# scverse/muon

Measured on AMD Instinct MI355X. Metric: cells/sec for TF-IDF+LSI(k=50), higher is better.
Workload: dtype f32

## Files before the change

### include/muon_amd.h

```cpp
#ifndef MUON_AMD_H
#define MUON_AMD_H

#include <stddef.h>
#include <stdint.h>

#ifdef __cplusplus
extern "C" {
#endif

typedef enum {
  MU_OK = 0,
  MU_ERR_ARG = -1,
  MU_ERR_HIP = -2,
  MU_ERR_NO_DEVICE = -3,
  MU_ERR_UNSUPPORTED = -4
} mu_status;

#define MU_DTYPE_F32 0
#define MU_DTYPE_F64 1

#define MU_TFIDF_LOG_TF 1
#define MU_TFIDF_LOG_IDF 2
#define MU_TFIDF_LOG_TFIDF 4

// ... 56 lines not shown
                                const float* d_values, const double* d_rowsum, const float* d_idf, double scale,
                                int flags, float* d_out, unsigned long long* d_zero_count, void* d_work,
                                size_t work_bytes, int have_slab_ptr, const int64_t* d_slab_ptr,
                                const int64_t* d_row_dst, void* d_ent, void* stream);
int mu_csr_slab_ptr(int64_t n_rows, int64_t n_cols, const int64_t* d_indptr, const int32_t* d_indices, int64_t* d_sp,
                    void* stream);
int mu_csr_slab_ptr_width(int64_t n_rows, int64_t n_cols, int64_t width, const int64_t* d_indptr,
                          const int32_t* d_indices, int64_t* d_sp, void* stream);
int mu_csr_row_col_sums_sp(int dtype, int64_t n_rows, int64_t n_cols, const int64_t* d_indptr,
                           const int32_t* d_indices, const void* d_values, double* d_rowsum, double* d_colsum,
                           void* d_work, size_t work_bytes, const int64_t* d_slab_ptr, void* stream);
int mu_tfidf_scale_sweep_sp(int dtype, int64_t n_rows, int64_t n_cols, const int64_t* d_indptr,
                            const int32_t* d_indices, const void* d_values, const double* d_rowsum, const void* d_idf,
                            double scale, int flags, void* d_out, unsigned long long* d_zero_count,
                            const int64_t* d_slab_ptr, void* stream);
int mu_tpack4_supported(int64_t n_rows, int64_t n_cols, int64_t nnz);
int mu_tpack4_geometry(int64_t n_rows, int64_t n_cols, int64_t nnz, int64_t* rows_per_block, int* n_blocks,
                       int* tile_cols);
size_t mu_tpack4_worksize(int64_t n_rows, int64_t n_cols, int64_t nnz);
int mu_tpack4_count(int64_t n_rows, int64_t n_cols, int64_t nnz, const int64_t* d_indptr, const int32_t* d_indices,
                    int64_t* d_col_nnz, void* d_work, size_t work_bytes, const int64_t* d_slab_ptr, void* stream);
int mu_tpack4_fill_stream(int64_t n_rows, int64_t n_cols, int64_t nnz, const int64_t* d_indptr,
                          const int32_t* d_indices, const float* d_values, const int64_t* d_x_row_dst,
                          const void* d_x_ent, const int64_t* d_sptr, const int32_t* d_inv, void* d_ent, void* d_work,
                          size_t work_bytes, void* stream);
int mu_tpack4_fill_csr(int64_t n_rows, int64_t n_cols, int64_t nnz, const int64_t* d_indptr, const int32_t* d_indices,
                       const float* d_values, const int64_t* d_x_row_dst, const void* d_x_ent,
                       const int64_t* d_t_indptr, int32_t* d_t_indices, float* d_t_values, void* d_work,
                       size_t work_bytes, void* stream);
int mu_tpack4_status(const void* d_work, int64_t n_rows, int64_t n_cols, int64_t nnz, int* h_err);
size_t mu_tpack4_err_offset(int64_t n_rows, int64_t n_cols, int64_t nnz);
size_t mu_tpack4_cnt_offset(int64_t n_rows, int64_t n_cols, int64_t nnz);
int mu_tpack4_phase_cycles(unsigned long long* h_out6, int reset);
int mu_csr_stream_len(int64_t n_pos, const int32_t* d_perm, const int64_t* d_indptr, int64_t* d_len,
                      void* stream);
int mu_csr_stream_fill(int64_t n_pos, const int32_t* d_perm, const int64_t* d_indptr,
                       const int32_t* d_indices, const float* d_values, const int64_t* d_sptr,
                       void* d_ent, void* stream);
int mu_spmm_stream_f32(int64_t n_pos, int64_t n_cols, const int64_t* d_sptr, const void* d_ent,
                       const int32_t* d_perm, int k_layout, const float* d_Q, int B, float* d_Y,
                       void* stream);
int mu_csr_slice_stream(int n_ranges, const int64_t* h_row0, const int64_t* h_rows, const int64_t* h_lo,
                        const int64_t* h_hi, int64_t n_cols, const int64_t* d_indptr, const int32_t* d_indices,
                        const float* d_values, const int64_t* d_slab_ptr, int64_t* d_sptr, void* d_ent, uint32_t* d_rel,
                        void* stream);
int mu_spmm_stream_ranges_f32(int64_t n_pos, const int64_t* d_sptr, const void* d_ent, const int32_t* d_perm,
                              int k_layout, const float* d_Q, int64_t q_rows, float* d_Y, int64_t y_stride,
                              const uint32_t* d_tbl, int64_t tbl_stride, int n_ranges, const int32_t* h_ranges5,
                              int per_wg, void* stream);
int mu_spmm_stream_f64(int64_t n_pos, int64_t n_cols, const int64_t* d_sptr, const void* d_ent,
                       const int32_t* d_perm, int k_layout, const double* d_Q, int B, double* d_Y,
                       int accumulate, void* stream);


int mu_spmm_ell16_waves(int64_t n_rows);
int mu_spmm_ell16_f32(int waves, int64_t n_pos, int64_t n_cols, const int32_t* d_hdr, const int64_t* d_wave_base,
                      const void* d_ent, const int32_t* d_perm, const float* d_Q, float* d_Y, void* stream);
int mu_spmm_ell16_f64(int waves, int64_t n_pos, int64_t n_cols, const int32_t* d_hdr, const int64_t* d_wave_base,
                      const void* d_ent, const int32_t* d_perm, const double* d_Q, double* d_Y, int accumulate,
                      void* stream);
int mu_spmm_ell16_parts(int64_t n_rows, int64_t n_cols, int wide, int* waves, int* parts);
int mu_spmm_ell16_parts_f32(int waves, int parts, int64_t n_pos, int64_t n_cols, const int32_t* d_hdr,
                            const int64_t* d_wave_base, const void* d_ent, const int32_t* d_perm, const float* d_Q,
                            float* d_Y, int64_t y_stride, void* stream);
int mu_spmm_ell16_parts_f64(int waves, int parts, int64_t n_pos, int64_t n_cols, const int32_t* d_hdr,
                            const int64_t* d_wave_base, const void* d_ent, const int32_t* d_perm, const double* d_Q,
// ... 135 lines not shown
```

### muon_amd/_backend.py

```python
from __future__ import annotations

from dataclasses import dataclass
from typing import Optional, Tuple

import contextlib
import os

import numpy as np
import torch

from . import _ffi
from ._ffi import F32, F64, check


@dataclass
class DeviceCSR:

    indptr: torch.Tensor
    indices: torch.Tensor
    values: torch.Tensor
    shape: Tuple[int, int]

    @property
    def nnz(self) -> int:
# ... 594 lines not shown
        self._tpack4_err = work[off:off + 4].view(torch.int32).clone()

    def take_tpack4_err(self):
        return self.__dict__.pop("_tpack4_err", None)

    @staticmethod
    def raise_tpack4(err: int) -> None:
        if int(err) != 0:
            raise _ffi.MuonAmdError(f"mu_tpack4_fill: the transposition tripped an internal invariant (error word {int(err)}: "
                                    "1 = bitmap and count pass disagree, 2 = a tile could not be narrowed); X^T would be wrong")

    def tpack4_status(self) -> int:
        import ctypes as C

        got = self.__dict__.get("_tpack4_work")
        if got is None:
            return 0
        work, (n, d, nnz) = got
        err = C.c_int(0)
        check(self.lib.mu_tpack4_status(_p(work), n, d, nnz, C.byref(err)))
        return int(err.value)

    def transpose_stream(self, X: DeviceCSR, sort_rows: bool = True, before_fill=None,
                         K: Optional[int] = None, src=None) -> DeviceStream:
        n, d = X.shape
        assert X.values.dtype == torch.float32
        col_nnz = self.empty((max(d, 1),), torch.int64)
        plan = self._plan_of(X, "tplan") if (sort_rows and K is None and self._use_tpack4(X)) else None
        if plan is not None:
            ent = self.empty((max(X.nnz, 1),), torch.int64)
            if before_fill is not None:
                before_fill()
            xs_ent, xs_dst = (src[0].ent, src[1]) if src is not None else (None, None)
            with self._dev_ctx():
                check(self.lib.mu_tpack4_fill_stream(n, d, X.nnz, _p(X.indptr), _p(X.indices), _p(X.values),
                                                     _p(xs_dst), _p(xs_ent), _p(plan["sptr"]), _p(plan["inv"]), _p(ent),
                                                     _p(plan["work"]), plan["wb"], self._stream()))
            self._note_tpack4(plan["work"], n, d, X.nnz)
            return DeviceStream(plan["sptr"], ent, (d, n), X.nnz, plan["perm"], plan["K"], self._t4_prefix(plan["work"], n, d, X.nnz))
        if self._use_tpack4(X):
            wb = int(self.lib.mu_tpack4_worksize(n, d, X.nnz))
            work = self.empty((wb,), torch.uint8)
            with self._dev_ctx():
                st = self._stream()
                check(self.lib.mu_tpack4_count(n, d, X.nnz, _p(X.indptr), _p(X.indices), _p(col_nnz), _p(work), wb,
                                               _p(self._slab_ptr_of(X)), st))
                want_k = K
                perm, inv, K, n_pos = None, None, max(1, int(want_k or self.lib.mu_spmm_stream_k(d))), d
                lens = col_nnz[:d]
                if sort_rows and d > 0:
                    perm, inv, K = self.launch_layout(lens, want_k)
                    n_pos = int(perm.numel())
                    plens = torch.zeros((n_pos,), dtype=torch.int64, device=self.device)
                    plens[inv.long()] = lens
                else:
                    plens = lens.contiguous()
                sptr = self._stream_sptr(plens, K)
                ent = self.empty((max(X.nnz, 1),), torch.int64)
                if before_fill is not None:
                    before_fill()
                xs_ent, xs_dst = (src[0].ent, src[1]) if src is not None else (None, None)
                check(self.lib.mu_tpack4_fill_stream(n, d, X.nnz, _p(X.indptr), _p(X.indices), _p(X.values),
                                                     _p(xs_dst), _p(xs_ent), _p(sptr), _p(inv), _p(ent), _p(work), wb, st))
            self._note_tpack4(work, n, d, X.nnz)
            return DeviceStream(sptr, ent, (d, n), X.nnz, perm, K, self._t4_prefix(work, n, d, X.nnz))
        if before_fill is not None:
            before_fill()
        return self.stream(self.transpose(X), sort_rows=sort_rows, K=K)

    def _t4_geometry(self, n, d, nnz):
        import ctypes as C

        rpb, G, Ct = C.c_int64(0), C.c_int(0), C.c_int(0)
        check(self.lib.mu_tpack4_geometry(n, d, nnz, C.byref(rpb), C.byref(G), C.byref(Ct)))
        return int(rpb.value), int(G.value)

    def _t4_prefix(self, work, n, d, nnz):
        rpb, G = self._t4_geometry(n, d, nnz)
        off = int(self.lib.mu_tpack4_cnt_offset(n, d, nnz))
        cnt = work[off:off + 4 * (G + 1) * d].view(torch.int32)
        return dict(cnt=cnt, rpb=rpb, blocks=G, stride=d)

    def slice_plan(self, X: DeviceCSR, n_s: int, max_ranges: int = 16):
        n, d = X.shape
        if n_s <= 0 or X.values.dtype != torch.float32 or not self._use_tpack4(X) or self._slab_ptr_of(X) is None:
            return None
        key = (X.indptr.data_ptr(), X.indices.data_ptr(), n, d, X.nnz, int(n_s), int(max_ranges))
        shared = self._plan_of(X, "tplan")
        got = shared.get("wplan") if shared is not None else getattr(X, "wplan", None)
        if got is not None and got[1] == key:
            return got[0]
        rpb, G = self._t4_geometry(n, d, X.nnz)
        if G < 1:
            return None
        blocks = max(1, min(G, int(round(n_s / rpb))))
        R = max(1, min(int(max_ranges), blocks))
        per = max(1, min(int(round(blocks / R)), G // R))
        g0s = [(r * G) // R for r in range(R)]
        rows = [(g0 * rpb, min((g0 + per) * rpb, n)) for g0 in g0s]
        edges = X.indptr[torch.tensor([v for ab in rows for v in ab], device=X.indptr.device)].tolist()
        plan = dict(rpb=rpb, ranges=[dict(g0=g0, g1=g0 + per, row0=a, row1=b, lo=int(edges[2 * i]), hi=int(edges[2 * i + 1]))
# ... 647 lines not shown
```

### muon_amd/_ffi.py

```python
from __future__ import annotations

import ctypes as C
import os
import threading

_HERE = os.path.dirname(os.path.abspath(__file__))
LIB_PATH = os.path.join(_HERE, "csrc", "libmuon_amd.so")

F32, F64 = 0, 1
TFIDF_LOG_TF, TFIDF_LOG_IDF, TFIDF_LOG_TFIDF = 1, 2, 4


class MuonAmdError(RuntimeError):
    pass


_lib = None
_lock = threading.Lock()

_i64, _i32, _dbl, _vp, _sz, _u64 = C.c_int64, C.c_int, C.c_double, C.c_void_p, C.c_size_t, C.c_uint64

SIGNATURES = {
    "mu_version": (C.c_int, []),
    "mu_last_error": (C.c_char_p, []),
# ... 13 lines not shown
    "mu_tfidf_scale": (C.c_int, [_i32, _i64, _vp, _vp, _vp, _vp, _vp, _dbl, _i32, _vp, _vp, _vp]),
    "mu_tfidf_scale_sweep": (C.c_int, [_i32, _i64, _i64, _vp, _vp, _vp, _vp, _vp, _dbl, _i32, _vp, _vp, _vp,
                                       _sz, _i32, _vp]),
    "mu_csr_count_nonzero": (C.c_int, [_i32, _i64, _vp, _vp, _vp, _vp]),
    "mu_csr_compact_nonzero": (C.c_int, [_i32, _i64, _vp, _vp, _vp, _vp, _vp, _vp, _vp]),
    "mu_exclusive_scan_i64": (C.c_int, [_i64, _vp, _vp, _vp]),
    "mu_binarize_values": (C.c_int, [_i32, _i64, _vp, _vp]),
    "mu_csr_transpose_worksize": (_sz, [_i64, _i64, _i64]),
    "mu_csr_transpose": (C.c_int, [_i32, _i64, _i64, _i64, _vp, _vp, _vp, _vp, _vp, _vp, _vp, _sz, _vp]),
    "mu_spmm_f32": (C.c_int, [_i64, _i64, _vp, _vp, _vp, _vp, _i32, _vp, _i32, _vp]),
    "mu_spmm_stream_k": (C.c_int, [_i64]),
    "mu_tfidf_scale_sweep_stream": (C.c_int, [_i64, _i64, _vp, _vp, _vp, _vp, _vp, _dbl, _i32, _vp, _vp, _vp, _sz, _i32,
                                              _vp, _vp, _vp, _vp]),
    "mu_csr_slab_ptr": (C.c_int, [_i64, _i64, _vp, _vp, _vp, _vp]),
    "mu_csr_slab_ptr_width": (C.c_int, [_i64, _i64, _i64, _vp, _vp, _vp, _vp]),
    "mu_csr_row_col_sums_sp": (C.c_int, [_i32, _i64, _i64, _vp, _vp, _vp, _vp, _vp, _vp, _sz, _vp, _vp]),
    "mu_tfidf_scale_sweep_sp": (C.c_int, [_i32, _i64, _i64, _vp, _vp, _vp, _vp, _vp, _dbl, _i32, _vp, _vp, _vp, _vp]),
    "mu_tpack4_supported": (C.c_int, [_i64, _i64, _i64]),
    "mu_tpack4_geometry": (C.c_int, [_i64, _i64, _i64, C.POINTER(_i64), C.POINTER(C.c_int), C.POINTER(C.c_int)]),
    "mu_tpack4_worksize": (_sz, [_i64, _i64, _i64]),
    "mu_tpack4_count": (C.c_int, [_i64, _i64, _i64, _vp, _vp, _vp, _vp, _sz, _vp, _vp]),
    "mu_tpack4_fill_stream": (C.c_int, [_i64, _i64, _i64, _vp, _vp, _vp, _vp, _vp, _vp, _vp, _vp, _vp, _sz, _vp]),
    "mu_tpack4_fill_csr": (C.c_int, [_i64, _i64, _i64, _vp, _vp, _vp, _vp, _vp, _vp, _vp, _vp, _vp, _sz, _vp]),
    "mu_tpack4_status": (C.c_int, [_vp, _i64, _i64, _i64, C.POINTER(C.c_int)]),
    "mu_tpack4_err_offset": (_sz, [_i64, _i64, _i64]),
    "mu_tpack4_phase_cycles": (C.c_int, [_vp, _i32]),
    "mu_csr_stream_len": (C.c_int, [_i64, _vp, _vp, _vp, _vp]),
    "mu_csr_stream_fill": (C.c_int, [_i64, _vp, _vp, _vp, _vp, _vp, _vp, _vp]),
    "mu_spmm_stream_f32": (C.c_int, [_i64, _i64, _vp, _vp, _vp, _i32, _vp, _i32, _vp, _vp]),
    "mu_spmm_stream_f64": (C.c_int, [_i64, _i64, _vp, _vp, _vp, _i32, _vp, _i32, _vp, _i32, _vp]),
    "mu_csr_slice_stream": (C.c_int, [_i32, _vp, _vp, _vp, _vp, _i64, _vp, _vp, _vp, _vp, _vp, _vp, _vp, _vp]),
    "mu_spmm_stream_ranges_f32": (C.c_int, [_i64, _vp, _vp, _vp, _i32, _vp, _i64, _vp, _i64, _vp, _i64, _i32, _vp, _i32, _vp]),
    "mu_tpack4_cnt_offset": (_sz, [_i64, _i64, _i64]),
    "mu_spmm_ell16_waves": (C.c_int, [_i64]),
    "mu_dense_col_moments_chunks": (C.c_int, [_i64, _i64]),
    "mu_dense_col_moments": (C.c_int, [_i32, _i64, _i64, _i64, _vp, _i32, _vp, _vp]),
    "mu_ell16_fill": (C.c_int, [_i64, _i64, _i64, _i32, _vp, _vp, _vp, _vp, _vp, _vp, _vp, _vp]),
    "mu_spmm_ell16_f32": (C.c_int, [_i32, _i64, _i64, _vp, _vp, _vp, _vp, _vp, _vp, _vp]),
    "mu_spmm_ell16_f64": (C.c_int, [_i32, _i64, _i64, _vp, _vp, _vp, _vp, _vp, _vp, _i32, _vp]),
    "mu_spmm_ell16_parts": (C.c_int, [_i64, _i64, _i32, C.POINTER(C.c_int), C.POINTER(C.c_int)]),
    "mu_spmm_ell16_parts_f32": (C.c_int, [_i32, _i32, _i64, _i64, _vp, _vp, _vp, _vp, _vp, _vp, _i64, _vp]),
    "mu_spmm_ell16_parts_f64": (C.c_int, [_i32, _i32, _i64, _i64, _vp, _vp, _vp, _vp, _vp, _vp, _i64, _vp]),
    "mu_tune_set": (C.c_int, [C.c_char_p, _i32]),
    "mu_tune_get": (C.c_int, [C.c_char_p]),
    "mu_spmm_f64": (C.c_int, [_i64, _i64, _vp, _vp, _vp, _vp, _i32, _vp, _i32, _vp]),
    "mu_gram_worksize": (_sz, [_i64, _i32]),
    "mu_gram_f32": (C.c_int, [_i64, _i32, _vp, _vp, _vp, _vp, _sz, _vp]),
    "mu_gram_cross_f32": (C.c_int, [_i64, _i32, _vp, _vp, _vp, _vp, _sz, _vp]),
    "mu_dense_apply_f32": (C.c_int, [_i64, _i32, _vp, _vp, _vp, _vp, _vp]),
    "mu_dense_project_out_f32": (C.c_int, [_i64, _i32, _vp, _vp, _vp, _vp]),
    "mu_chol_rinv_f64": (C.c_int, [_i32, _i32, _vp, _vp, _vp, _vp]),
    "mu_randn_f32": (C.c_int, [_i64, _u64, _vp, _vp]),
    "mu_skinny_tn_worksize": (_sz, [_i32, _i64, _i64]),
    "mu_skinny_nn": (C.c_int, [_i32, _i64, _i64, _i64, _vp, _vp, _vp, _vp]),
    "mu_skinny_tn": (C.c_int, [_i32, _i64, _i64, _i64, _vp, _vp, _vp, _vp, _sz, _vp]),
    "mu_skinny_nn_f64_f32": (C.c_int, [_i64, _i64, _i64, _vp, _vp, _vp, _vp]),
    "mu_skinny_tn_f64_f32": (C.c_int, [_i64, _i64, _i64, _vp, _vp, _vp, _vp, _sz, _vp]),
    "mu_mofa_update_w": (C.c_int, [_i32, _i64, _i32, _i32] + [_vp] * 7 + [_i32] + [_vp] * 6),
    "mu_mofa_update_z": (C.c_int, [_i32, _i64, _i32, _i32, _i32] + [_vp] * 11),
    "mu_mofa_rowstats_work_doubles": (_sz, [_i32]),
    "mu_mofa_rowstats": (C.c_int, [_i32, _i64, _i64, _i32, _vp, _vp, _vp, _vp, _i32, _vp, _i32, _i32, _vp, _i64,
                                   _vp, _vp, _vp, _vp, _vp]),
    "mu_umap_strengths_f64": (C.c_int, [_i64, _i32, _vp, _vp, _dbl, _dbl, _vp, _vp]),
    "mu_wnn_bandwidth_f64": (C.c_int, [_i64, _i32, _vp, _vp, _vp, _vp, _vp, _i32, _dbl, _vp, _vp, _vp]),
    "mu_knn_filter_f64": (C.c_int, [_i64, _i64, _i64, _i32] + [_vp] * 6 + [_i32] + [_vp] * 4),
    "mu_knn_merge_f64": (C.c_int, [_i64, _i32, _i32] + [_vp] * 9),
# ... 72 lines not shown
```

### muon_amd/csrc/build.py

```python
#!/usr/bin/env python
import hashlib
import os
import subprocess
import sys

HERE = os.path.dirname(os.path.abspath(__file__))
ROOT = os.path.dirname(os.path.dirname(HERE))
SOURCES = ["runtime.hip", "tfidf.hip", "transpose.hip", "spmm.hip", "spmm_win.hip", "spmm_narrow.hip", "spmm_ell.hip", "tpack4.hip", "dense.hip", "skinny.hip", "synth.hip", "mofa.hip", "mofa_elbo.hip", "mofa_stats.hip", "mofa_poisson.hip", "mofa_bernoulli.hip", "knn.hip", "wnn.hip"]
HEADERS = ["common.hpp", "sweep.hpp", os.path.join(ROOT, "include", "muon_amd.h")]
_VGPR_FORM = ["-mllvm", "-amdgpu-mfma-vgpr-form"]
EXTRA = {"skinny.hip": _VGPR_FORM, "dense.hip": _VGPR_FORM, "knn.hip": _VGPR_FORM, "mofa_poisson.hip": _VGPR_FORM, "mofa_bernoulli.hip": _VGPR_FORM}
LIB = os.path.join(HERE, "libmuon_amd.so")
ARCH = "gfx950"
FLAGS = ["-O3", "-std=c++17", "-fPIC", f"--offload-arch={ARCH}", "-I" + os.path.join(ROOT, "include"),
         "-I" + HERE, "-Wall", "-Wno-unused-function"]


def _hipcc():
    for cand in (os.environ.get("HIPCC"), "/opt/rocm/bin/hipcc", "hipcc"):
        if cand and (os.path.isabs(cand) and os.path.exists(cand) or not os.path.isabs(cand)):
            return cand
    raise RuntimeError("hipcc not found")


def _digest(paths):
    h = hashlib.sha256()
    for p in paths:
        with open(p, "rb") as f:
            h.update(f.read())
    h.update(" ".join(f for f in FLAGS if not f.startswith("-I")).encode())
    h.update(repr(sorted(EXTRA.items())).encode())
    h.update(_compiler_id().encode())
    return h.hexdigest()


def _compiler_id():
    try:
        out = subprocess.run([_hipcc(), "--version"], capture_output=True, text=True, timeout=30).stdout
        return " | ".join(l.strip() for l in out.splitlines() if "version" in l.lower())[:300]
    except Exception:
        return ""
# ... 36 lines not shown
```

### muon_amd/csrc/runtime.hip

```cpp
#include <atomic>
#include <cstdarg>
#include <cstdio>
#include <cstring>
#include <thread>
#include <vector>
#include "common.hpp"

static thread_local char g_err[512] = "";

void mu_set_error(const char* fmt, ...) {
  va_list ap;
  va_start(ap, fmt);
  vsnprintf(g_err, sizeof(g_err), fmt, ap);
  va_end(ap);
}

int mu_num_cus() {
  static int cached[64] = {0};
  int dev = 0;
  if (hipGetDevice(&dev) != hipSuccess || dev < 0 || dev >= 64) return 256;
  if (cached[dev] == 0) {
    int n = 0;
    if (hipDeviceGetAttribute(&n, hipDeviceAttributeMultiprocessorCount, dev) != hipSuccess ||
        n <= 0)
      n = 256;
    cached[dev] = n;
  }
  return cached[dev];
}

static const char* const kTuneKeys[] = {"spmm_k", "spmm_mode", "gram_wg", "pack_wg", "tpack_dbg", "spmm_narrow_off", "ell_mode", "tfidf_wide", "tfidf_pipe", "nn_interleave", "tfidf_abl", "tfidf_sum_m", "tn_pipe", "nn_fast_off", "stream_pipe", "tpack4_m", "tpack4_c", "scale_stream_off", "tpack4_plain", "tpack4_abl", "tpack4_late", "tpack4_circ", "tpack4_off", "pois_valu", "pois_lane"};
constexpr int kTuneN = sizeof(kTuneKeys) / sizeof(kTuneKeys[0]);
static int g_tune[kTuneN] = {};

extern "C" {

int mu_version(void) { return 601; }

int mu_tune_set(const char* key, int value) {
  MU_REQUIRE(key, "null key");
  for (int i = 0; i < kTuneN; ++i)
    if (strcmp(key, kTuneKeys[i]) == 0) {
      MU_REQUIRE(value >= 0, "negative value");
      MU_REQUIRE(i != 0 || value <= 16, "spmm_k must be 0..16");
      g_tune[i] = value;
      return MU_OK;
    }
  mu_set_error("mu_tune_set: unknown key %s", key);
  return MU_ERR_ARG;
}

int mu_tune_get(const char* key) {
  if (key)
    for (int i = 0; i < kTuneN; ++i)
      if (strcmp(key, kTuneKeys[i]) == 0) return g_tune[i];
  return -1;
}

const char* mu_last_error(void) { return g_err; }

int mu_device_count(int* count) {
  MU_REQUIRE(count, "null count");
  int n = 0;
  hipError_t e = hipGetDeviceCount(&n);
// ... 120 lines not shown
```

Before: 3.450 million.

## Add precomputed tile permutation plan for transpose-stream fill from row stream

Adds a new tperm kernel pair. A one-time plan pass records column tiles, overflow continuation lanes and per-entry staging slots. A move kernel then transposes the already-packed row stream of X into the column stream using those cached slots, with inline-asm pipelined loads and a double-buffered LDS staging area. The goal is to skip the per-call counting, sorting and bitmap work of the tpack4 fill when the plan is reused across calls. The cost is extra memory for the plan (a 16-bit slot per nnz), heavy register-pinned inline assembly, and a fallback path when alignment or plan preconditions fail.

```diff
diff --git a/include/muon_amd.h b/include/muon_amd.h
--- a/include/muon_amd.h
+++ b/include/muon_amd.h
@@ -112,6 +112,13 @@
 size_t mu_tpack4_err_offset(int64_t n_rows, int64_t n_cols, int64_t nnz);
 size_t mu_tpack4_cnt_offset(int64_t n_rows, int64_t n_cols, int64_t nnz);
 int mu_tpack4_phase_cycles(unsigned long long* h_out6, int reset);
+int mu_tperm_stage_pairs(void);
+int mu_tperm_plan(int64_t n_rows, int64_t n_cols, int64_t nnz, const int64_t* d_indptr, const int32_t* d_indices,
+                  const int64_t* d_x_row_dst, int tile_cols, const int64_t* d_tile_off, int32_t* d_ntile,
+                  int32_t* d_tiles, uint32_t* d_cont, uint16_t* d_slots, void* stream);
+int mu_tperm_fill(int64_t n_rows, int64_t n_cols, int64_t nnz, const int64_t* d_indptr, const int64_t* d_x_row_dst,
+                  const void* d_x_ent, const int64_t* d_cdst, const void* d_cnt, const int64_t* d_tile_off,
+                  const int32_t* d_tiles, const uint32_t* d_cont, const uint16_t* d_slots, void* d_ent, void* stream);
 int mu_csr_stream_len(int64_t n_pos, const int32_t* d_perm, const int64_t* d_indptr, int64_t* d_len,
                       void* stream);
 int mu_csr_stream_fill(int64_t n_pos, const int32_t* d_perm, const int64_t* d_indptr,
diff --git a/muon_amd/_backend.py b/muon_amd/_backend.py
--- a/muon_amd/_backend.py
+++ b/muon_amd/_backend.py
@@ -650,10 +650,17 @@
             if before_fill is not None:
                 before_fill()
             xs_ent, xs_dst = (src[0].ent, src[1]) if src is not None else (None, None)
+            tp = self._tperm_of(X, plan, xs_ent, xs_dst) if src is not None else None
             with self._dev_ctx():
-                check(self.lib.mu_tpack4_fill_stream(n, d, X.nnz, _p(X.indptr), _p(X.indices), _p(X.values),
-                                                     _p(xs_dst), _p(xs_ent), _p(plan["sptr"]), _p(plan["inv"]), _p(ent),
-                                                     _p(plan["work"]), plan["wb"], self._stream()))
+                if tp is not None:
+                    cnt = plan["work"][int(self.lib.mu_tpack4_cnt_offset(n, d, X.nnz)):]
+                    check(self.lib.mu_tperm_fill(n, d, X.nnz, _p(X.indptr), _p(xs_dst), _p(xs_ent), _p(tp["cdst"]), _p(cnt),
+                                                 _p(tp["toff"]), _p(tp["tiles"]), _p(tp["cont"]), _p(tp["slots"]), _p(ent),
+                                                 self._stream()))
+                else:
+                    check(self.lib.mu_tpack4_fill_stream(n, d, X.nnz, _p(X.indptr), _p(X.indices), _p(X.values),
+                                                         _p(xs_dst), _p(xs_ent), _p(plan["sptr"]), _p(plan["inv"]), _p(ent),
+                                                         _p(plan["work"]), plan["wb"], self._stream()))
             self._note_tpack4(plan["work"], n, d, X.nnz)
             return DeviceStream(plan["sptr"], ent, (d, n), X.nnz, plan["perm"], plan["K"], self._t4_prefix(plan["work"], n, d, X.nnz))
         if self._use_tpack4(X):
@@ -685,6 +692,46 @@
         if before_fill is not None:
             before_fill()
         return self.stream(self.transpose(X), sort_rows=sort_rows, K=K)
+
+    def _tperm_of(self, X: DeviceCSR, plan, xs_ent, xs_dst):
+        import ctypes as C
+
+        lib = self.lib
+        if plan.get("tperm") is False:
+            return None
+        xplan = self._plan_of(X, "xplan")
+        if (lib.mu_tune_get(b"tperm_off") == 1 or lib.mu_tune_get(b"tpack_dbg") > 0 or xplan is None
+                or xs_dst is not xplan["row_dst"] or xs_ent.data_ptr() % 256 != 0):
+            return None
+        n, d = X.shape
+        got = plan.get("tperm")
+        keys = (lib.mu_tune_get(b"tpack4_c"), lib.mu_tune_get(b"tpack4_m"))
+        if got is not None and got["keys"] == keys:
+            return got
+        rpb, G, Ct = C.c_int64(0), C.c_int(0), C.c_int(0)
+        check(lib.mu_tpack4_geometry(n, d, X.nnz, C.byref(rpb), C.byref(G), C.byref(Ct)))
+        G, Ct = int(G.value), min(int(Ct.value), 512)
+        try:
+            with self._dev_ctx():
+                st = self._stream()
+                ntile = self.empty((G,), torch.int32)
+                check(lib.mu_tperm_plan(n, d, X.nnz, _p(X.indptr), _p(X.indices), None, Ct, None, _p(ntile), None, None,
+                                        None, st))
+                toff = torch.zeros((G + 1,), dtype=torch.int64, device=self.device)
+                toff[1:] = torch.cumsum(ntile.long(), 0)
+                T = int(toff[-1].item())
+                tiles = self.empty((T + G,), torch.int32)
+                cont = self.empty((16 * T,), torch.int32)
+                slots = self.empty((X.nnz,), torch.int16)
+                check(lib.mu_tperm_plan(n, d, X.nnz, _p(X.indptr), _p(X.indices), _p(xs_dst), Ct, _p(toff), None,
+                                        _p(tiles), _p(cont), _p(slots), st))
+                inv = plan["inv"]
+                cdst = (plan["sptr"][inv.long()] if inv is not None else plan["sptr"][:d]).contiguous()
+        except (RuntimeError, MemoryError):
+            plan["tperm"] = False
+            return None
+        plan["tperm"] = dict(keys=keys, tile_cols=Ct, toff=toff, tiles=tiles, cont=cont, slots=slots, cdst=cdst, n_tiles=T)
+        return plan["tperm"]
 
     def _t4_geometry(self, n, d, nnz):
         import ctypes as C
diff --git a/muon_amd/_ffi.py b/muon_amd/_ffi.py
--- a/muon_amd/_ffi.py
+++ b/muon_amd/_ffi.py
@@ -69,6 +69,9 @@
     "mu_csr_slice_stream": (C.c_int, [_i32, _vp, _vp, _vp, _vp, _i64, _vp, _vp, _vp, _vp, _vp, _vp, _vp, _vp]),
     "mu_spmm_stream_ranges_f32": (C.c_int, [_i64, _vp, _vp, _vp, _i32, _vp, _i64, _vp, _i64, _vp, _i64, _i32, _vp, _i32, _vp]),
     "mu_tpack4_cnt_offset": (_sz, [_i64, _i64, _i64]),
+    "mu_tperm_stage_pairs": (C.c_int, []),
+    "mu_tperm_plan": (C.c_int, [_i64, _i64, _i64, _vp, _vp, _vp, _i32, _vp, _vp, _vp, _vp, _vp, _vp]),
+    "mu_tperm_fill": (C.c_int, [_i64, _i64, _i64, _vp, _vp, _vp, _vp, _vp, _vp, _vp, _vp, _vp, _vp, _vp]),
     "mu_spmm_ell16_waves": (C.c_int, [_i64]),
     "mu_dense_col_moments_chunks": (C.c_int, [_i64, _i64]),
     "mu_dense_col_moments": (C.c_int, [_i32, _i64, _i64, _i64, _vp, _i32, _vp, _vp]),
diff --git a/muon_amd/csrc/build.py b/muon_amd/csrc/build.py
--- a/muon_amd/csrc/build.py
+++ b/muon_amd/csrc/build.py
@@ -6,7 +6,7 @@
 
 HERE = os.path.dirname(os.path.abspath(__file__))
 ROOT = os.path.dirname(os.path.dirname(HERE))
-SOURCES = ["runtime.hip", "tfidf.hip", "transpose.hip", "spmm.hip", "spmm_win.hip", "spmm_narrow.hip", "spmm_ell.hip", "tpack4.hip", "dense.hip", "skinny.hip", "synth.hip", "mofa.hip", "mofa_elbo.hip", "mofa_stats.hip", "mofa_poisson.hip", "mofa_bernoulli.hip", "knn.hip", "wnn.hip"]
+SOURCES = ["runtime.hip", "tfidf.hip", "transpose.hip", "spmm.hip", "spmm_win.hip", "spmm_narrow.hip", "spmm_ell.hip", "tpack4.hip", "tperm.hip", "dense.hip", "skinny.hip", "synth.hip", "mofa.hip", "mofa_elbo.hip", "mofa_stats.hip", "mofa_poisson.hip", "mofa_bernoulli.hip", "knn.hip", "wnn.hip"]
 HEADERS = ["common.hpp", "sweep.hpp", os.path.join(ROOT, "include", "muon_amd.h")]
 _VGPR_FORM = ["-mllvm", "-amdgpu-mfma-vgpr-form"]
 EXTRA = {"skinny.hip": _VGPR_FORM, "dense.hip": _VGPR_FORM, "knn.hip": _VGPR_FORM, "mofa_poisson.hip": _VGPR_FORM, "mofa_bernoulli.hip": _VGPR_FORM}
diff --git a/muon_amd/csrc/runtime.hip b/muon_amd/csrc/runtime.hip
--- a/muon_amd/csrc/runtime.hip
+++ b/muon_amd/csrc/runtime.hip
@@ -29,7 +29,7 @@
   return cached[dev];
 }
 
-static const char* const kTuneKeys[] = {"spmm_k", "spmm_mode", "gram_wg", "pack_wg", "tpack_dbg", "spmm_narrow_off", "ell_mode", "tfidf_wide", "tfidf_pipe", "nn_interleave", "tfidf_abl", "tfidf_sum_m", "tn_pipe", "nn_fast_off", "stream_pipe", "tpack4_m", "tpack4_c", "scale_stream_off", "tpack4_plain", "tpack4_abl", "tpack4_late", "tpack4_circ", "tpack4_off", "pois_valu", "pois_lane"};
+static const char* const kTuneKeys[] = {"spmm_k", "spmm_mode", "gram_wg", "pack_wg", "tpack_dbg", "spmm_narrow_off", "ell_mode", "tfidf_wide", "tfidf_pipe", "nn_interleave", "tfidf_abl", "tfidf_sum_m", "tn_pipe", "nn_fast_off", "stream_pipe", "tpack4_m", "tpack4_c", "scale_stream_off", "tpack4_plain", "tpack4_abl", "tpack4_late", "tpack4_circ", "tpack4_off", "tperm_off", "pois_valu", "pois_lane"};
 constexpr int kTuneN = sizeof(kTuneKeys) / sizeof(kTuneKeys[0]);
 static int g_tune[kTuneN] = {};
 
diff --git a/muon_amd/csrc/tperm.hip b/muon_amd/csrc/tperm.hip
--- /dev/null
+++ b/muon_amd/csrc/tperm.hip
@@ -0,0 +1,508 @@
+#include <type_traits>
+#include <utility>
+
+#include "common.hpp"
+#pragma clang diagnostic ignored "-Winline-asm"
+
+namespace {
+
+constexpr int kT = 1024, kNW = 16;
+constexpr int kMaxC = 512;
+constexpr int kCap = 9216;
+constexpr int kH0 = 72;
+constexpr int kW0 = 76;
+constexpr int kS0 = 110;
+constexpr int kSlotP = 16;
+constexpr int kNone = 0xff;
+
+#define MU_TP_CLOB                                                                                                      \
+  "v72", "v73", "v74", "v75", "v76", "v77", "v78", "v79", "v80", "v81", "v82", "v83", "v84", "v85", "v86", "v87", "v88", \
+      "v89", "v90", "v91", "v92", "v93", "v94", "v95", "v96", "v97", "v98", "v99", "v100", "v101", "v102", "v103",       \
+      "v104", "v105", "v106", "v107", "v108", "v109", "v110", "v111", "v112", "v113", "v114", "v115", "v116", "v117",    \
+      "v118", "v119", "v120", "v121", "v122", "v123", "v124", "v125", "v126", "v127"
+
+template <int L>
+__device__ __forceinline__ int tp_writelane_c(int v, int x) {
+  asm("v_writelane_b32 %0, %1, %2" : "+v"(v) : "s"(x), "n"(L));
+  return v;
+}
+__device__ __forceinline__ int tp_writelane_s(int v, int x, int l) {
+  asm("s_mov_b32 m0, %2\n\tv_writelane_b32 %0, %1, m0" : "+v"(v) : "s"(x), "s"(l) : "m0");
+  return v;
+}
+__device__ __forceinline__ uint64_t tp_readlane_u64(uint64_t v, int l) {
+  const unsigned lo = (unsigned)__builtin_amdgcn_readlane((int)(unsigned)v, l);
+  const unsigned hi = (unsigned)__builtin_amdgcn_readlane((int)(unsigned)(v >> 32), l);
+  return ((uint64_t)hi << 32) | lo;
+}
+__device__ __forceinline__ int tp_wave_min(int v) {
+#pragma unroll
+  for (int off = 32; off > 0; off >>= 1) {
+    const int t = __shfl_xor(v, off, 64);
+    v = t < v ? t : v;
+  }
+  return v;
+}
+
+template <bool REC>
+__global__ __launch_bounds__(kT) void k_tperm_plan(int64_t n_rows, int64_t n_cols, int Cmax, int rw,
+                                                   const int64_t* __restrict__ indptr,
+                                                   const int32_t* __restrict__ indices,
+                                                   const int64_t* __restrict__ row_dst,
+                                                   const int64_t* __restrict__ toff, int32_t* __restrict__ ntile,
+                                                   int32_t* __restrict__ tiles, uint32_t* __restrict__ cont,
+                                                   uint16_t* __restrict__ slots) {
+  __shared__ uint32_t bm[REC ? kNW : 1][kMaxC];
+  __shared__ uint32_t fs[REC ? kNW : 1][kMaxC];
+  __shared__ uint32_t wsum[kNW];
+  __shared__ int s_lim;
+  __shared__ unsigned s_tot;
+  const int g = blockIdx.x;
+  const int tid = threadIdx.x, lane = tid & 63, wave = tid >> 6, sub = lane & 31;
+  const int64_t rpb = (int64_t)kNW * rw;
+  const int64_t r0 = (int64_t)g * rpb;
+  const int64_t r1 = (r0 + rpb) < n_rows ? (r0 + rpb) : n_rows;
+  const int64_t row = r0 + (int64_t)wave * rw + sub;
+  const bool active = lane < 32 && sub < rw && row < r1;
+  int64_t cur = active ? indptr[row] : 0;
+  const int64_t end = active ? indptr[row + 1] : 0;
+  const int64_t dst0 = (REC && active) ? row_dst[row] - cur : 0;
+  if (REC)
+    for (int t = tid; t < kNW * kMaxC; t += kT) (&bm[0][0])[t] = 0u;
+  const int64_t tb = REC ? toff[g] + g : 0, tc = REC ? toff[g] : 0;
+  int t = 0;
+  for (int64_t cb = 0; cb < n_cols; ++t) {
+    if (tid == 0) {
+      s_lim = (int)((cb + Cmax) < n_cols ? (cb + Cmax) : n_cols);
+      s_tot = 0u;
+    }
+    __syncthreads();
+    const int64_t left = end - cur;
+    int x = left > 32 ? indices[cur + 32] : 0x7fffffff;
+    int lim = tp_wave_min(left > 64 ? indices[cur + 64] : 0x7fffffff);
+#pragma unroll
+    for (int k = 0; k < 2; ++k) {
+      const int m = tp_wave_min(x);
+      const unsigned long long b = __ballot(x == m);
+      if (lane == (int)__builtin_ctzll(b)) x = 0x7fffffff;
+    }
+    const int m3 = tp_wave_min(x);
+    lim = m3 < lim ? m3 : lim;
+    if (lane == 0 && lim != 0x7fffffff) atomicMin(&s_lim, lim);
+    __syncthreads();
+    int cend = s_lim;
+    int n;
+    unsigned total;
+    for (;;) {
+      int lo = 0, hi = (int)(left < 64 ? left : 64);
+      while (lo < hi) {
+        const int mid = (lo + hi) >> 1;
+        if (indices[cur + mid] < cend) lo = mid + 1; else hi = mid;
+      }
+      n = lo;
+      const int ws = wave_sum_all(n);
+      if (lane == 0 && ws) atomicAdd(&s_tot, (unsigned)ws);
+      __syncthreads();
+      total = s_tot;
+      __syncthreads();
+      if (total <= (unsigned)kCap) break;
+      if (tid == 0) s_tot = 0u;
+      int w = ((int)(cend - cb) / 2 / 16) * 16;
+      w = w < 16 ? 16 : w;
+      cend = (int)cb + w;
+      __syncthreads();
+    }
+    if (REC) {
+      if (tid == 0) tiles[tb + t] = (int32_t)cb;
+      const unsigned over = (unsigned)__ballot(n > 32);
+      if (lane == 0) {
+        int pa = kNone, pb = kNone;
+        if (over) {
+          pa = __builtin_ctz(over);
+          const unsigned o2 = over & (over - 1u);
+          if (o2) pb = __builtin_ctz(o2);
+        }
+        cont[(tc + t) * kNW + wave] = (uint32_t)(pa | (pb << 8));
+      }
+      if (total > 0u) {
+        const int W = cend - (int)cb;
+        for (int k = 0; k < n; ++k) atomicOr(&bm[wave][indices[cur + k] - (int)cb], 1u << sub);
+        __syncthreads();
+        uint32_t mine = 0;
+        if (tid < W)
+          for (int w = 0; w < kNW; ++w) mine += (uint32_t)__popc(bm[w][tid]);
+        uint32_t incl = mine;
+#pragma unroll
+        for (int off = 1; off < 64; off <<= 1) {
+          const uint32_t u = __shfl_up(incl, off, 64);
+          if (lane >= off) incl += u;
+        }
+        if (lane == 63) wsum[wave] = incl;
+        __syncthreads();
+        uint32_t run = incl - mine;
+        for (int w = 0; w < wave; ++w) run += wsum[w];
+        if (tid < W)
+          for (int w = 0; w < kNW; ++w) {
+            fs[w][tid] = run;
+            run += (uint32_t)__popc(bm[w][tid]);
+          }
+        __syncthreads();
+        for (int k = 0; k < n; ++k) {
+          const int c = indices[cur + k] - (int)cb;
+          slots[dst0 + cur + k] = (uint16_t)(fs[wave][c] + (uint32_t)__popc(bm[wave][c] & ((1u << sub) - 1u)));
+        }
+        __syncthreads();
+        if (tid < W)
+          for (int w = 0; w < kNW; ++w) bm[w][tid] = 0u;
+      }
+    }
+    cur += n;
+    cb = cend;
+  }
+  if (tid == 0) {
+    if (REC) tiles[tb + t] = (int32_t)n_cols;
+    else ntile[g] = t;
+  }
+}
+
+template <int J>
+__device__ __forceinline__ void tp_issue_circ(uint64_t b0, uint64_t b1, uint64_t tb0, uint64_t tb1, unsigned s0, unsigned s1,
+                                              unsigned m0, unsigned m1, unsigned sub, unsigned sub8, unsigned sub8w,
+                                              unsigned sub2, unsigned sub2w) {
+  unsigned long long save;
+  unsigned p0, p1, q0, q1;
+  asm volatile(
+      "s_mov_b64 %[save], exec\n\t"
+      "v_cmp_gt_u32 vcc, %[s0], %[sub]\n\t"
+      "v_cndmask_b32 %[p0], %[sub8], %[sub8w], vcc\n\t"
+      "v_cndmask_b32 %[q0], %[sub2], %[sub2w], vcc\n\t"
+      "v_cmp_gt_u32 vcc, %[s1], %[sub]\n\t"
+      "v_cndmask_b32 %[p1], %[sub8], %[sub8w], vcc\n\t"
+      "v_cndmask_b32 %[q1], %[sub2], %[sub2w], vcc\n\t"
+      "s_mov_b32 exec_lo, %[m0]\n\t"
+      "s_mov_b32 exec_hi, 0\n\t"
+      "global_load_dwordx2 v[%c[C]:%c[V]], %[p0], %[b0]\n\t"
+      "global_load_ushort v%c[S], %[q0], %[tb0]\n\t"
+      "s_mov_b32 exec_lo, 0\n\t"
+      "s_mov_b32 exec_hi, %[m1]\n\t"
+      "global_load_dwordx2 v[%c[C]:%c[V]], %[p1], %[b1]\n\t"
+      "global_load_ushort v%c[S], %[q1], %[tb1]\n\t"
+      "s_mov_b64 exec, %[save]"
+      : [save] "=&s"(save), [p0] "=&v"(p0), [p1] "=&v"(p1), [q0] "=&v"(q0), [q1] "=&v"(q1)
+      : [sub] "v"(sub), [sub8] "v"(sub8), [sub8w] "v"(sub8w), [sub2] "v"(sub2), [sub2w] "v"(sub2w), [b0] "s"(b0),
+        [b1] "s"(b1), [tb0] "s"(tb0), [tb1] "s"(tb1), [s0] "s"(s0), [s1] "s"(s1), [m0] "s"(m0), [m1] "s"(m1),
+        [C] "i"(kW0 + 2 * J), [V] "i"(kW0 + 2 * J + 1), [S] "i"(kS0 + J)
+      : MU_TP_CLOB, "vcc", "memory");
+}
+__device__ __forceinline__ void tp_issue_cont(uint64_t a0, uint64_t a1, uint64_t t0, uint64_t t1, int n0, int n1,
+                                              unsigned sub8, unsigned sub2) {
+  unsigned long long save, m0, m1;
+  asm volatile(
+      "s_bfm_b64 %[m0], %[n0], 0\n\t"
+      "s_bfm_b64 %[m1], %[n1], 32\n\t"
+      "s_mov_b64 %[save], exec\n\t"
+      "v_mov_b32 v%c[C], 0x7fffffff\n\t"
+      "s_mov_b64 exec, %[m0]\n\t"
+      "global_load_dwordx2 v[%c[C]:%c[V]], %[o8], %[a0]\n\t"
+      "global_load_ushort v%c[S], %[o2], %[t0]\n\t"
+      "s_mov_b64 exec, %[m1]\n\t"
+      "global_load_dwordx2 v[%c[C]:%c[V]], %[o8], %[a1]\n\t"
+      "global_load_ushort v%c[S], %[o2], %[t1]\n\t"
+      "s_mov_b64 exec, %[save]"
+      : [save] "=&s"(save), [m0] "=&s"(m0), [m1] "=&s"(m1)
+      : [o8] "v"(sub8), [o2] "v"(sub2), [a0] "s"(a0), [a1] "s"(a1), [t0] "s"(t0), [t1] "s"(t1), [n0] "s"(n0), [n1] "s"(n1),
+        [C] "i"(kW0 + 2 * kSlotP), [V] "i"(kW0 + 2 * kSlotP + 1), [S] "i"(kS0 + kSlotP)
+      : MU_TP_CLOB, "memory");
+}
+template <int J>
+__device__ __forceinline__ void tp_pad_slot() {
+  asm volatile("v_mov_b32 v%c0, 0x7fffffff" ::"i"(kW0 + 2 * J) : MU_TP_CLOB);
+}
+template <int J>
+__device__ __forceinline__ void tp_retire_slot(int cend, int pad) {
+  asm volatile(
+      "v_cmp_le_i32 vcc, %0, v%c1\n\t"
+      "v_cndmask_b32 v%c1, %2, v%c1, vcc" ::"s"(cend),
+      "i"(kW0 + 2 * J), "v"(pad)
+      : MU_TP_CLOB, "vcc");
+}
+__device__ __forceinline__ void tp_wait_all() { asm volatile("s_waitcnt vmcnt(0)" ::: MU_TP_CLOB, "memory"); }
+template <int R>
+__device__ __forceinline__ unsigned tp_reg() {
+  unsigned v;
+  asm volatile("v_mov_b32 %0, v%c1" : "=v"(v) : "i"(R) : MU_TP_CLOB);
+  return v;
+}
+__device__ __forceinline__ void tp_issue_header(const uint32_t* bg, const uint32_t* bn, const int64_t* cd, unsigned off4) {
+  asm volatile(
+      "global_load_dword v%c4, %0, %1\n\t"
+      "global_load_dword v%c5, %0, %2\n\t"
+      "v_lshlrev_b32 v%c6, 1, %0\n\t"
+      "global_load_dwordx2 v[%c6:%c7], v%c6, %3"
+      :
+      : "v"(off4), "s"(bg), "s"(bn), "s"(cd), "i"(kH0), "i"(kH0 + 1), "i"(kH0 + 2), "i"(kH0 + 3)
+      : MU_TP_CLOB, "memory");
+}
+
+template <int... I, class F>
+__device__ __forceinline__ void tp_for_impl(std::integer_sequence<int, I...>, F&& f) {
+  (f(std::integral_constant<int, I>{}), ...);
+}
+template <int N, class F>
+__device__ __forceinline__ void tp_for(F&& f) {
+  tp_for_impl(std::make_integer_sequence<int, N>{}, static_cast<F&&>(f));
+}
+
+__global__ __launch_bounds__(kT) __attribute__((amdgpu_num_vgpr(36))) void k_tperm_move(
+    int64_t n_rows, int64_t n_cols, int rw, int G, const int64_t* __restrict__ indptr,
+    const int64_t* __restrict__ row_dst, const unsigned long long* __restrict__ xent,
+    const int64_t* __restrict__ cdst, const uint32_t* __restrict__ base, const int64_t* __restrict__ toff,
+    const int32_t* __restrict__ tiles, const uint32_t* __restrict__ cont, const uint16_t* __restrict__ slots,
+    unsigned long long* __restrict__ out) {
+  __shared__ unsigned long long stage[2][kCap];
+  __shared__ uint32_t lrun[2][kMaxC];
+  __shared__ int64_t gdst[2][kMaxC];
+  __shared__ uint32_t wsum[2][kNW];
+  int g = blockIdx.x;
+  if (G > 0) {
+    const int per = (G + 7) / 8;
+    g = (g % 8) * per + (g / 8);
+    if (g >= G) return;
+  } else {
+    G = -G;
+  }
+  const int tid = threadIdx.x, lane = tid & 63;
+  const int wave = uniform32(tid >> 6);
+  const int half = lane >> 5, sub = lane & 31;
+  const int64_t rpb = (int64_t)kNW * rw;
+  const int64_t r0 = (int64_t)g * rpb;
+  const int64_t r1 = (r0 + rpb) < n_rows ? (r0 + rpb) : n_rows;
+  const int64_t wr0 = r0 + (int64_t)wave * rw;
+
+  uint64_t A = 0;
+  int rem = 0, ld = 0;
+  {
+    const int64_t row = wr0 + sub;
+    const bool ok = sub < rw && row < r1;
+    const int64_t p0 = ok ? indptr[row] : 0;
+    rem = ok ? (int)(indptr[row + 1] - p0) : 0;
+    A = (uint64_t)xent + 8ull * (uint64_t)(ok ? row_dst[row] : 0);
+  }
+  const int64_t tb = uniform64(toff[g]) + g;
+  const int nt = (int)(uniform64(toff[g + 1]) - uniform64(toff[g]));
+  const uint32_t* cw = cont + (tb - g) * kNW + wave;
+  const unsigned subo = (unsigned)sub * 8u, sub2 = (unsigned)sub * 2u;
+  tp_for<16>([&](auto jc) { tp_pad_slot<decltype(jc)::value>(); });
+
+  auto cont_of = [&](int t) { return t < nt ? uniform32((int)cw[(int64_t)t * kNW]) : (kNone | (kNone << 8)); };
+  auto issue_all = [&](int pw) {
+    const int remc = rem < 32 ? rem : 32;
+    const int nn = remc - ld;
+    const uint64_t st = A + 8ull * (uint64_t)(unsigned)ld;
+    const unsigned s5 = (unsigned)(st >> 3) & 31u;
+    const unsigned rot = __builtin_rotateleft32((unsigned)((1ull << nn) - 1ull), s5);
+    const uint64_t b256 = st & ~255ull;
+    const uint64_t tb64 = (uint64_t)slots + ((b256 - (uint64_t)xent) >> 2);
+    ld = remc;
+    tp_for<16>([&](auto jc) {
+      constexpr int J = decltype(jc)::value;
+      tp_issue_circ<J>(tp_readlane_u64(b256, 2 * J), tp_readlane_u64(b256, 2 * J + 1), tp_readlane_u64(tb64, 2 * J),
+                       tp_readlane_u64(tb64, 2 * J + 1), (unsigned)__builtin_amdgcn_readlane((int)s5, 2 * J),
+                       (unsigned)__builtin_amdgcn_readlane((int)s5, 2 * J + 1),
+                       (unsigned)__builtin_amdgcn_readlane((int)rot, 2 * J),
+                       (unsigned)__builtin_amdgcn_readlane((int)rot, 2 * J + 1), (unsigned)sub, subo, subo + 256u, sub2,
+                       sub2 + 64u);
+    });
+    const int pa = pw & 0xff, pb = pw >> 8;
+    if (pa != kNone) {
+      const int lb = pb != kNone ? pb : pa;
+      int na = __builtin_amdgcn_readlane(rem, pa) - 32, nb = pb != kNone ? __builtin_amdgcn_readlane(rem, pb) - 32 : 0;
+      na = __builtin_amdgcn_readfirstlane(na < 0 ? 0 : (na > 32 ? 32 : na));
+      nb = __builtin_amdgcn_readfirstlane(nb < 0 ? 0 : (nb > 32 ? 32 : nb));
+      const uint64_t a0 = tp_readlane_u64(A, pa) + 256u, a1 = tp_readlane_u64(A, lb) + 256u;
+      tp_issue_cont(a0, a1, (uint64_t)slots + ((a0 - (uint64_t)xent) >> 2), (uint64_t)slots + ((a1 - (uint64_t)xent) >> 2),
+                    na, nb, subo, sub2);
+    }
+  };
+  const uint32_t* base_g = base + (int64_t)g * n_cols;
+  const uint32_t* base_n = base + (int64_t)(g + 1) * n_cols;
+  auto issue_header = [&](int64_t cb) {
+    int64_t ofs = n_cols - 1 - cb;
+    if (ofs < 0) {
+      ofs = 0;
+      cb = n_cols - 1;
+    }
+    const unsigned o4 = (unsigned)((int64_t)tid < ofs ? (int64_t)tid : ofs) * 4u;
+    tp_issue_header(base_g + cb, base_n + cb, cdst + cb, o4);
+  };
+  uint32_t mine = 0, incl = 0;
+  int64_t gd = 0;
+  auto take_header = [&](int W, int set) {
+    const uint32_t b0 = tp_reg<kH0>(), b1 = tp_reg<kH0 + 1>();
+    const unsigned lo = tp_reg<kH0 + 2>(), hi = tp_reg<kH0 + 3>();
+    mine = tid < W ? b1 - b0 : 0u;
+    gd = (int64_t)(((unsigned long long)hi << 32) | lo) + (int64_t)b0;
+    incl = mine;
+#pragma unroll
+    for (int off = 1; off < 64; off <<= 1) {
+      const uint32_t u = __shfl_up(incl, off, 64);
+      if (lane >= off) incl += u;
+    }
+    if (lane == 63) wsum[set][wave] = incl;
+  };
+  auto finish_header = [&](int W, int set) {
+    uint32_t wpre = 0;
+#pragma unroll
+    for (int w = 0; w < kNW; ++w) {
+      const uint32_t u = wsum[set][w];
+      if (w < wave) wpre += u;
+    }
+    if (tid < W) {
+      lrun[set][tid] = (mine << 16) | (wpre + incl - mine);
+      gdst[set][tid] = gd;
+    }
+  };
+  auto write_out = [&](int set, int ncol) {
+    const unsigned long long* stg = stage[set];
+    const int grp = tid >> 4, s16 = tid & 15;
+    for (int c0 = grp; c0 < ncol; c0 += 4 * (kT / 16)) {
+      uint32_t lr[4];
+      int64_t gq[4];
+      unsigned long long e[4];
+#pragma unroll
+      for (int u = 0; u < 4; ++u) {
+        const int cl = c0 + u * (kT / 16);
+        const bool in = cl < ncol;
+        lr[u] = in ? lrun[set][in ? cl : 0] : 0u;
+        gq[u] = gdst[set][in ? cl : 0];
+      }
+#pragma unroll
+      for (int u = 0; u < 4; ++u) {
+        const uint32_t L = lr[u] >> 16, src = lr[u] & 0xffffu;
+        e[u] = stg[(uint32_t)s16 < L ? src + s16 : 0];
+      }
+#pragma unroll
+      for (int u = 0; u < 4; ++u) {
+        const uint32_t L = lr[u] >> 16, src = lr[u] & 0xffffu;
+        if ((uint32_t)s16 < L) out[gq[u] + s16] = e[u];
+        for (uint32_t i = 16 + s16; i < L; i += 16) out[gq[u] + i] = stg[src + i];
+      }
+    }
+  };
+
+  auto tile_at = [&](int t) { return uniform32(tiles[tb + (t < nt ? t : nt)]); };
+  int c0 = tile_at(0), c1 = tile_at(1), c2 = tile_at(2);
+  issue_header(c0);
+  tp_wait_all();
+  take_header(c1 - c0, 0);
+  int pw = cont_of(0);
+  issue_all(pw);
+  issue_header(c1);
+  __syncthreads();
+  finish_header(c1 - c0, 0);
+
+  for (int t = 0; t < nt; ++t) {
+    const int set = t & 1;
+    const int cend = c1;
+    int hf = half;
+    asm volatile("" : "+v"(hf));
+    const int pw_next = cont_of(t + 1);
+    tp_wait_all();
+    take_header(c2 - c1, set ^ 1);
+    unsigned long long* stg = stage[set];
+    int cntv = 0;
+    tp_for<16>([&](auto jc) {
+      constexpr int J = decltype(jc)::value;
+      const int c = (int)tp_reg<kW0 + 2 * J>();
+      const unsigned v = tp_reg<kW0 + 2 * J + 1>(), s = tp_reg<kS0 + J>();
+      const bool valid = c < cend;
+      const unsigned long long m = __ballot(valid);
+      if (valid) stg[s] = (unsigned long long)(unsigned)(wr0 + 2 * J + hf) | ((unsigned long long)v << 32);
+      cntv = tp_writelane_c<2 * J>(cntv, __popc((unsigned)m));
+      cntv = tp_writelane_c<2 * J + 1>(cntv, __popc((unsigned)(m >> 32)));
+    });
+    const int pa = pw & 0xff, pb = pw >> 8;
+    if (pa != kNone) {
+      const int lb = pb != kNone ? pb : pa;
+      const int c = (int)tp_reg<kW0 + 2 * kSlotP>();
+      const unsigned v = tp_reg<kW0 + 2 * kSlotP + 1>(), s = tp_reg<kS0 + kSlotP>();
+      const bool valid = c < cend;
+      const unsigned long long m = __ballot(valid);
+      if (valid) stg[s] = (unsigned long long)(unsigned)(wr0 + (hf ? lb : pa)) | ((unsigned long long)v << 32);
+      cntv = tp_writelane_s(cntv, __builtin_amdgcn_readlane(cntv, pa) + __popc((unsigned)m), pa);
+      if (pb != kNone) cntv = tp_writelane_s(cntv, __builtin_amdgcn_readlane(cntv, pb) + __popc((unsigned)(m >> 32)), pb);
+    }
+    {
+      int padv = 0x7fffffff;
+      asm volatile("" : "+v"(padv));
+      tp_for<16>([&](auto jc) { tp_retire_slot<decltype(jc)::value>(cend, padv); });
+    }
+    if (half == 0) {
+      A += (uint64_t)(unsigned)cntv * 8u;
+      rem -= cntv;
+      ld = ld > cntv ? ld - cntv : 0;
+    }
+    pw = pw_next;
+    issue_all(pw);
+    issue_header(c2);
+    const int c3 = tile_at(t + 3);
+    __syncthreads();
+    finish_header(c2 - c1, set ^ 1);
+    write_out(set, c1 - c0);
+    c0 = c1;
+    c1 = c2;
+    c2 = c3;
+  }
+  tp_wait_all();
+}
+
+}
+
+extern "C" {
+
+int mu_tperm_stage_pairs(void) { return kCap; }
+
+int mu_tperm_plan(int64_t n_rows, int64_t n_cols, int64_t nnz, const int64_t* d_indptr, const int32_t* d_indices,
+                  const int64_t* d_x_row_dst, int tile_cols, const int64_t* d_tile_off, int32_t* d_ntile,
+                  int32_t* d_tiles, uint32_t* d_cont, uint16_t* d_slots, void* stream) {
+  MU_REQUIRE(mu_tpack4_supported(n_rows, n_cols, nnz), "shape out of range (mu_tpack4_supported)");
+  MU_REQUIRE(d_indptr && d_indices, "null pointer");
+  MU_REQUIRE(tile_cols >= 16 && tile_cols <= kMaxC, "tile_cols out of range (16 .. 512)");
+  MU_REQUIRE(d_tile_off ? (d_x_row_dst && d_tiles && d_cont && d_slots) : d_ntile != nullptr,
+             "count pass: d_ntile; record pass: d_x_row_dst, d_tile_off, d_tiles, d_cont, d_slots");
+  int64_t rpb = 0;
+  int G = 0;
+  mu_tpack4_geometry(n_rows, n_cols, nnz, &rpb, &G, nullptr);
+  const int rw = (int)(rpb / kNW);
+  hipStream_t st = (hipStream_t)stream;
+  if (d_tile_off)
+    hipLaunchKernelGGL((k_tperm_plan<true>), dim3(G), dim3(kT), 0, st, n_rows, n_cols, tile_cols, rw, d_indptr, d_indices,
+                       d_x_row_dst, d_tile_off, d_ntile, d_tiles, d_cont, d_slots);
+  else
+    hipLaunchKernelGGL((k_tperm_plan<false>), dim3(G), dim3(kT), 0, st, n_rows, n_cols, tile_cols, rw, d_indptr,
+                       d_indices, d_x_row_dst, d_tile_off, d_ntile, d_tiles, d_cont, d_slots);
+  MU_CHECK_LAUNCH();
+  return MU_OK;
+}
+
+int mu_tperm_fill(int64_t n_rows, int64_t n_cols, int64_t nnz, const int64_t* d_indptr, const int64_t* d_x_row_dst,
+                  const void* d_x_ent, const int64_t* d_cdst, const void* d_cnt, const int64_t* d_tile_off,
+                  const int32_t* d_tiles, const uint32_t* d_cont, const uint16_t* d_slots, void* d_ent, void* stream) {
+  MU_REQUIRE(mu_tpack4_supported(n_rows, n_cols, nnz), "shape out of range (mu_tpack4_supported)");
+  MU_REQUIRE(d_indptr && d_x_row_dst && d_x_ent && d_cdst && d_cnt && d_tile_off && d_tiles && d_cont && d_slots && d_ent,
+             "null pointer");
+  MU_REQUIRE((reinterpret_cast<uintptr_t>(d_x_ent) & 255) == 0, "the row stream of X must be 256-byte aligned");
+  int64_t rpb = 0;
+  int G = 0;
+  mu_tpack4_geometry(n_rows, n_cols, nnz, &rpb, &G, nullptr);
+  const int rw = (int)(rpb / kNW);
+  const bool xcd = mu_tune_get("tpack4_plain") != 1;
+  const unsigned grid = xcd ? (unsigned)(8 * ((G + 7) / 8)) : (unsigned)G;
+  hipLaunchKernelGGL(k_tperm_move, dim3(grid), dim3(kT), 0, (hipStream_t)stream, n_rows, n_cols, rw, xcd ? G : -G,
+                     d_indptr, d_x_row_dst, (const unsigned long long*)d_x_ent, d_cdst, (const uint32_t*)d_cnt, d_tile_off,
+                     d_tiles, d_cont, d_slots, (unsigned long long*)d_ent);
+  MU_CHECK_LAUNCH();
+  return MU_OK;
+}
+
+}
```

Measured after the change: 3.516 million, median of 6. 1.9% higher.
